# JackAILab/ConsistentID

Hardware: AMD Instinct MI355X
Metric: 512x512 SD1.5 images/sec/node @50 DDIM steps (higher is better)
Workload: dtype f16; 1 GPU; sd15 ConsistentID 512x512, 50 DDIM steps, batch 4/GPU (global 4), CFG batch 8, LoRA rank 128 merged, start_merge_step 30, hipGraph on; global_batch=4, parallelism=dp1 (images sharded, no in-step collective)

## Files before the change

### consistentid_amd/csrc/attn.hip

```cpp
#include "common.h"
#include "../../include/cid.h"
#include <stdlib.h>
#include <type_traits>

#ifndef CID_ATTN_ABL
#define CID_ATTN_ABL 0
#endif
#ifdef CID_ATTN_MAX_AT_HEAD
#define CID_ATTN_HEADMAX true
#else
#define CID_ATTN_HEADMAX false
#endif

namespace {

__device__ __forceinline__ float max17f(float m, const f32x16& v) {
#pragma unroll
    for (int r = 0; r < 16; r += 2) m = __builtin_fmaxf(__builtin_fmaxf(m, v[r]), v[r + 1]);
    return m;
}

template <int D, int QT, int NWV>
struct AttnCfg {
    static constexpr int NT = 64 * NWV;
    static constexpr int BQ = 32 * QT * NWV;
    static constexpr int DKP = (D + 15) / 16 * 16;
    static constexpr int KSTEPS = DKP / 16;
    static constexpr int DVT = (D + 31) / 32;
    static constexpr int NCH = D / 8;
    static constexpr int CR = DVT * 32 - D;
    static constexpr int KBYTES = (DKP / 8) * 1024;
    static constexpr int VDATA = D * 128;
    static constexpr int VBYTES = VDATA + CR * 128;
    static constexpr int BUF = KBYTES + VBYTES;
    static constexpr int PPW = (NCH + NWV - 1) / NWV;
};

template <int D, int QT, int NWV, bool MASK, bool CAUSAL = false>
__global__ void __launch_bounds__(64 * NWV, (QT == 1 && D <= 40 && NWV == 4) ? 3 : ((QT == 1 && D <= 80) ? 2 : 1))
self_attn_kernel(const half_t* __restrict__ q, const half_t* __restrict__ k, const half_t* __restrict__ vt,
                 half_t* __restrict__ out, int N, int heads, int ldq, int ldk, int dvp, int ldo, int n_keys, int xcd_remap) {
#if defined(__HIP_DEVICE_COMPILE__)
    using Cfg = AttnCfg<D, QT, NWV>;
    constexpr int NT = Cfg::NT, KSTEPS = Cfg::KSTEPS, DVT = Cfg::DVT;
    constexpr int NCH = Cfg::NCH, CR = Cfg::CR;
    extern __shared__ __attribute__((aligned(16))) char smem[];
    typedef __attribute__((address_space(3))) void lds_void;

    const int tid = threadIdx.x, lane = tid & 63;
    const int wave = __builtin_amdgcn_readfirstlane(tid >> 6);
    const int idx = lane & 31, hi = lane >> 5;
    int bid = blockIdx.x + gridDim.x * (blockIdx.y + gridDim.y * blockIdx.z);
    {
        const int nwg = gridDim.x * gridDim.y * gridDim.z;
        if (xcd_remap && (nwg & 7) == 0) bid = (bid & 7) * (nwg >> 3) + (bid >> 3);
    }
    const int bx = bid % (int)gridDim.x;
    const int h = (bid / (int)gridDim.x) % (int)gridDim.y, b = bid / (int)(gridDim.x * gridDim.y);
    const int q0 = bx * Cfg::BQ + wave * (32 * QT);

    const half_t* kbase = k + (long)b * N * ldk + h * D;
    const half_t* vbase = vt + ((long)(b * heads + h) * dvp) * N;

#if defined(CID_ATTN_NOBIAS)
    constexpr bool BIAS = false;
#else
    constexpr bool BIAS = Cfg::DKP > D;
#endif
    static_assert(!BIAS || Cfg::DKP - D == 8, "pad is one 16-byte slot");
    static_assert(!(CAUSAL && BIAS), "causal mode: the running max starts behind the mask (no bias slot)");
    if (Cfg::DKP > D) {
        half8 pad = zero_h8();
        if (BIAS) pad[0] = (half_t)1.f;
        for (int r = tid; r < 2 * 64; r += NT)
            *reinterpret_cast<half8*>(smem + (r >> 6) * Cfg::BUF + NCH * 1024 + (r & 63) * 16) = pad;
    }
    const bool bias_lane = BIAS && ((KSTEPS - 1) * 16 + hi * 8 == D);

    half8 qf[QT][KSTEPS];
#pragma unroll
    for (int t = 0; t < QT; ++t) {
        const half_t* qrow = q + ((long)b * N + q0 + t * 32 + idx) * ldq + h * D;
#pragma unroll
        for (int kk = 0; kk < KSTEPS; ++kk) {
            const int c = kk * 16 + hi * 8;
            qf[t][kk] = (c < D) ? ld_global_h8(qrow + c) : zero_h8();
        }
    }

    constexpr bool ONES = (D % 32) != 0;
    constexpr int ONES_REG = ((D % 32) & 3) + 4 * ((D % 32) >> 3);
    constexpr int ONES_HI = ((D % 32) >> 2) & 1;
    if (ONES) {
        half8 one;
#pragma unroll
        for (int i = 0; i < 8; ++i) one[i] = (half_t)1.f;
        for (int e = tid; e < 2 * 8 * CR; e += NT) {
            const int bf = e / (8 * CR), rem = e - bf * (8 * CR);
            *reinterpret_cast<half8*>(smem + bf * Cfg::BUF + Cfg::KBYTES + Cfg::VDATA + rem * 16) = one;
        }
    }

    const __amdgpu_buffer_rsrc_t rs_k = __builtin_amdgcn_make_buffer_rsrc((void*)kbase, 0, (unsigned)(((long)(N - 1) * ldk + D) * 2), 0x00020000);
    const __amdgpu_buffer_rsrc_t rs_v = __builtin_amdgcn_make_buffer_rsrc((void*)vbase, 0, (unsigned)((long)D * N * 2), 0x00020000);
    const unsigned kvo = (unsigned)(lane * ldk * 2);
    unsigned vvo[Cfg::PPW];
#pragma unroll
    for (int j = 0; j < Cfg::PPW; ++j) {
        const int sl = (j * NWV + wave) * 64 + lane;
        const int c = sl / D, r = sl - c * D;
        vvo[j] = (unsigned)(((long)r * N + c * 8) * 2);
    }
    auto dma_k = [&](int key0, int buf) {
#pragma unroll
        for (int j = 0; j < Cfg::PPW; ++j) {
            const int p = j * NWV + wave;
            if (p < NCH)
                __builtin_amdgcn_raw_ptr_buffer_load_lds(rs_k, (lds_void*)(smem + buf * Cfg::BUF + p * 1024), 16, kvo,
                                                         key0 * ldk * 2 + p * 16, 0, 0);
        }
    };
    auto dma_v = [&](int key0, int buf) {
#pragma unroll
        for (int j = 0; j < Cfg::PPW; ++j) {
            const int p = j * NWV + wave;
            if (p < NCH)
                __builtin_amdgcn_raw_ptr_buffer_load_lds(rs_v, (lds_void*)(smem + buf * Cfg::BUF + Cfg::KBYTES + p * 1024), 16,
                                                         vvo[j], key0 * 2, 0, 0);
        }
    };
    auto qk = [&](int buf, f32x16 (&s)[2][QT]) {
        const char* kb = smem + buf * Cfg::BUF;
#pragma unroll
        for (int kt = 0; kt < 2; ++kt)
#pragma unroll
            for (int t = 0; t < QT; ++t) s[kt][t] = zero_f16v();
#pragma unroll
        for (int kk = 0; kk < KSTEPS; ++kk) {
            half8 kf[2];
#pragma unroll
            for (int kt = 0; kt < 2; ++kt)
                kf[kt] = *reinterpret_cast<const half8*>(kb + (kk * 2 + hi) * 1024 + (kt * 32 + idx) * 16);
#pragma unroll
            for (int kt = 0; kt < 2; ++kt)
#pragma unroll
                for (int t = 0; t < QT; ++t) { if (!(CID_ATTN_ABL & 4)) s[kt][t] = mfma32(kf[kt], qf[t][kk], s[kt][t]); else s[kt][t][kk] += (float)kf[kt][0]; }
        }
    };
    const int vlane = (hi * D + idx) * 16;
    const int vlane_c = Cfg::VDATA + (hi * CR + idx + (DVT - 1) * 32 - D) * 16;
    const bool vconst_lane = (DVT - 1) * 32 + idx >= D;

    f32x16 oacc[DVT][QT];
#pragma unroll
    for (int d = 0; d < DVT; ++d)
#pragma unroll
        for (int t = 0; t < QT; ++t) oacc[d][t] = zero_f16v();
    float m_run[QT], l_run[QT];
#pragma unroll
    for (int t = 0; t < QT; ++t) { m_run[t] = -INFINITY; l_run[t] = 0.f; }

    const int ntiles = CAUSAL ? (min(n_keys, bx * Cfg::BQ + Cfg::BQ) + 63) / 64 : N / 64;
    dma_k(0, 0); dma_v(0, 0);
    if (ntiles > 1) dma_k(64, 1);
    asm volatile("s_waitcnt vmcnt(0)" ::: "memory");
    __syncthreads();
    f32x16 s_cur[2][QT], s_nxt[2][QT];
    qk(0, s_cur);
    auto tile_max = [&](f32x16 (&sc)[2][QT], int t) {
        float mx = max17f(sc[0][t][0], sc[0][t]);
        mx = max17f(mx, sc[1][t]);
        return fmaxf(mx, __shfl_xor(mx, 32, 64));
    };
    auto rebias = [&](f32x16 (&sc)[2][QT], int t, float m_new, float delta) {
        if (bias_lane) qf[t][KSTEPS - 1][0] = (half_t)(-m_new);
#pragma unroll
        for (int kt = 0; kt < 2; ++kt)
#pragma unroll
            for (int r = 0; r < 16; ++r) sc[kt][t][r] -= delta;
    };
    float mx_a[QT], mx_b[QT];
    if (MASK && BIAS && n_keys < 64) {
#pragma unroll
        for (int kt = 0; kt < 2; ++kt)
#pragma unroll
            for (int t = 0; t < QT; ++t)
#pragma unroll
                for (int r = 0; r < 16; ++r)
                    if (kt * 32 + crow(r, hi) >= n_keys) s_cur[kt][t][r] = -INFINITY;
    }
#pragma unroll
    for (int t = 0; t < QT; ++t) {
        const float mx = tile_max(s_cur, t);
        if (BIAS) {
            const float m0 = (float)(half_t)fminf(fmaxf(mx, -60000.f), 60000.f);
            rebias(s_cur, t, m0, m0);
            m_run[t] = m0;
            mx_a[t] = mx - m0;
        } else {
            mx_a[t] = mx;
        }
        mx_b[t] = 0.f;
    }
    __syncthreads();

    auto step = [&](int tile, auto has_next_tag, f32x16 (&s_cur)[2][QT], f32x16 (&s_nxt)[2][QT], float (&mx_cur)[QT],
                    float (&mx_nxt)[QT]) {
        constexpr bool HAS_NEXT = decltype(has_next_tag)::value;
        const int cur = tile & 1;
        if (!(CID_ATTN_ABL & 8)) {
            if (tile + 2 < ntiles) dma_k((tile + 2) * 64, cur);
            if (HAS_NEXT) dma_v((tile + 1) * 64, cur ^ 1);
        }
        if (MASK && (tile + 1) * 64 > n_keys) {
#pragma unroll
            for (int kt = 0; kt < 2; ++kt)
#pragma unroll
                for (int t = 0; t < QT; ++t)
#pragma unroll
                    for (int r = 0; r < 16; ++r)
                        if (tile * 64 + kt * 32 + crow(r, hi) >= n_keys) s_cur[kt][t][r] = -INFINITY;
        }
        if (CAUSAL && (tile * 64 + 63 > q0 || (tile + 1) * 64 > n_keys)) {
#pragma unroll
            for (int kt = 0; kt < 2; ++kt)
#pragma unroll
                for (int t = 0; t < QT; ++t)
#pragma unroll
                    for (int r = 0; r < 16; ++r) {
                        const int j = tile * 64 + kt * 32 + crow(r, hi);
                        if (j > q0 + t * 32 + idx || j >= n_keys) s_cur[kt][t][r] = -INFINITY;
                    }
        }
#pragma unroll
        for (int t = 0; t < QT; ++t) {
            const float mx = (CID_ATTN_ABL & 16) ? s_cur[0][t][0] : ((MASK || CAUSAL || CID_ATTN_HEADMAX) ? tile_max(s_cur, t) : mx_cur[t]);
            if (__any(mx > (BIAS ? 8.f : m_run[t] + 8.f))) {
                float m_new, alpha;
                if (BIAS) {
                    m_new = (float)(half_t)fminf(m_run[t] + fmaxf(mx, 0.f), 60000.f);
                    const float delta = m_new - m_run[t];
                    alpha = __builtin_amdgcn_exp2f(-delta);
                    rebias(s_cur, t, m_new, delta);
                } else {
                    m_new = fmaxf(m_run[t], mx);
                    alpha = __builtin_amdgcn_exp2f(m_run[t] - m_new);
                }
                m_run[t] = m_new;
                l_run[t] *= alpha;
#pragma unroll
                for (int d = 0; d < DVT; ++d)
#pragma unroll
                    for (int r = 0; r < 16; ++r) oacc[d][t][r] *= alpha;
            }
        }
        if (HAS_NEXT) qk(cur ^ 1, s_nxt);
        half8 pf[QT][4];
#pragma unroll
        for (int t = 0; t < QT; ++t) {
            const float m = m_run[t];
            float rs = 0.f;
#pragma unroll
            for (int kt = 0; kt < 2; ++kt)
#pragma unroll
                for (int g = 0; g < 2; ++g) {
                    half8 pv;
#pragma unroll
                    for (int i = 0; i < 8; ++i) {
                        const float a_ = BIAS ? s_cur[kt][t][g * 8 + i] : s_cur[kt][t][g * 8 + i] - m;
                        const float p = (CID_ATTN_ABL & 1) ? a_ * 0.001f : __builtin_amdgcn_exp2f(a_);
                        if (!ONES) rs += p;
                        pv[i] = (half_t)p;
                    }
                    pf[t][kt * 2 + g] = pv;
                }
            if (!ONES) l_run[t] += rs;
        }
        const char* vb = smem + cur * Cfg::BUF + Cfg::KBYTES;
#pragma unroll
        for (int ks = 0; ks < 4; ++ks) {
            half8 vf[DVT];
#pragma unroll
            for (int d = 0; d < DVT; ++d) {
                int off = vlane + (ks * 2 * D + d * 32) * 16;
                if (CR > 0 && d == DVT - 1) off = vconst_lane ? vlane_c + ks * 2 * CR * 16 : off;
                vf[d] = *reinterpret_cast<const half8*>(vb + off);
            }
#pragma unroll
            for (int d = 0; d < DVT; ++d)
#pragma unroll
                for (int t = 0; t < QT; ++t) { if (!(CID_ATTN_ABL & 2)) oacc[d][t] = mfma32(vf[d], pf[t][ks], oacc[d][t]); else oacc[d][t][ks] += (float)vf[d][0] * (float)pf[t][ks][0]; }
        }
        if (HAS_NEXT && !MASK && !CAUSAL && !CID_ATTN_HEADMAX) {
#pragma unroll
            for (int t = 0; t < QT; ++t) mx_nxt[t] = tile_max(s_nxt, t);
        }
        asm volatile("s_waitcnt vmcnt(0)" ::: "memory");
        __syncthreads();
    };
    int tile = 0;
    for (; tile + 2 < ntiles; tile += 2) {
        step(tile, std::true_type{}, s_cur, s_nxt, mx_a, mx_b);
        step(tile + 1, std::true_type{}, s_nxt, s_cur, mx_b, mx_a);
    }
    if (ntiles - tile == 2) {
        step(tile, std::true_type{}, s_cur, s_nxt, mx_a, mx_b);
        step(tile + 1, std::false_type{}, s_nxt, s_cur, mx_b, mx_a);
    } else {
        step(tile, std::false_type{}, s_cur, s_nxt, mx_a, mx_b);
    }

#pragma unroll
    for (int t = 0; t < QT; ++t) {
        float l;
        if (ONES) {
            const float mine = oacc[DVT - 1][t][ONES_REG];
            const float other = __shfl_xor(mine, 32, 64);
            l = (hi == ONES_HI) ? mine : other;
        } else {
            l = l_run[t] + __shfl_xor(l_run[t], 32, 64);
        }
        const float inv = 1.f / l;
        half_t* orow = out + ((long)b * N + q0 + t * 32 + idx) * ldo + h * D;
#pragma unroll
        for (int d = 0; d < DVT; ++d)
#pragma unroll
            for (int j = 0; j < 4; ++j) {
                const int dd = d * 32 + 8 * j + 4 * hi;
                if (dd < D) {
                    half4 o;
#pragma unroll
                    for (int i = 0; i < 4; ++i) o[i] = (half_t)(oacc[d][t][j * 4 + i] * inv);
                    *reinterpret_cast<half4*>(orow + dd) = o;
                }
            }
    }
#endif
}

template <int D, int QT, int NWV, bool MASK = false, bool CAUSAL = false>
int launch_attn(const half_t* q, const half_t* k, const half_t* vt, half_t* out, int B, int N, int heads,
                int ldq, int ldk, int dvp, int ldo, int n_keys, hipStream_t s) {
    using Cfg = AttnCfg<D, QT, NWV>;
    constexpr int smem = 2 * Cfg::BUF;
    static bool configured = false;
    auto kern = self_attn_kernel<D, QT, NWV, MASK, CAUSAL>;
    if (!configured) {
        hipError_t herr = hipFuncSetAttribute((const void*)kern, hipFuncAttributeMaxDynamicSharedMemorySize, smem);
        if (herr != hipSuccess) {
            cid_set_error("cid_self_attn_f16: cannot reserve %d bytes of LDS (%s)", smem, hipGetErrorString(herr));
            return -5;
        }
        configured = true;
    }
    dim3 grid(N / Cfg::BQ, heads, B);
    static int remap = -1;
    if (remap < 0) { const char* e = getenv("CID_ATTN_XCD"); remap = e ? atoi(e) : 1; }
    hipLaunchKernelGGL(kern, grid, dim3(Cfg::NT), smem, s, q, k, vt, out, N, heads, ldq, ldk, dvp, ldo, n_keys, remap);
    return 0;
}

}

extern "C" int cid_self_attn_f16(const cid_half* q, const cid_half* k, const cid_half* vt, cid_half* out,
                                 int32_t B, int32_t N, int32_t heads, int32_t d,
                                 int32_t ldq, int32_t ldk, int32_t dvp, int32_t ldo, cid_stream_t stream) {
    return cid_self_attn_keys_f16(q, k, vt, out, B, N, heads, d, ldq, ldk, dvp, ldo, N, stream);
}

extern "C" int cid_self_attn_keys_f16(const cid_half* q, const cid_half* k, const cid_half* vt, cid_half* out,
                                      int32_t B, int32_t N, int32_t heads, int32_t d, int32_t ldq, int32_t ldk,
                                      int32_t dvp, int32_t ldo, int32_t n_keys, cid_stream_t stream) {
    CID_CHECK_ARG(q && k && vt && out, "cid_self_attn_f16: null pointer");
    CID_CHECK_ARG(n_keys > 0 && n_keys <= N, "cid_self_attn_keys_f16: n_keys must be in (0, N] (got %d, N = %d)", n_keys, N);
    CID_CHECK_ARG(B > 0 && heads > 0 && N > 0 && N % 64 == 0, "cid_self_attn_f16: N must be a positive multiple of 64 (got %d)", N);
    CID_CHECK_ARG(ldq % 8 == 0 && ldk % 8 == 0 && ldo % 4 == 0 && dvp >= d, "cid_self_attn_f16: bad pitches");
    const half_t* Q = (const half_t*)q; const half_t* K = (const half_t*)k; const half_t* V = (const half_t*)vt;
    half_t* O = (half_t*)out;
    hipStream_t s = (hipStream_t)stream;
    int rc = -22;
#define CID_ATTN(DD, QT, NWV) rc = launch_attn<DD, QT, NWV>(Q, K, V, O, B, N, heads, ldq, ldk, dvp, ldo, n_keys, s)
#define CID_ATTN_MASKED(DD) \
    rc = (N % 128 == 0) ? launch_attn<DD, 1, 4, true>(Q, K, V, O, B, N, heads, ldq, ldk, dvp, ldo, n_keys, s) \
                        : launch_attn<DD, 1, 2, true>(Q, K, V, O, B, N, heads, ldq, ldk, dvp, ldo, n_keys, s)
    if (n_keys != N) {
        if (d == 80) CID_ATTN_MASKED(80);
        else if (d == 64) CID_ATTN_MASKED(64);
        else if (d == 40) CID_ATTN_MASKED(40);
        else if (d == 160) CID_ATTN_MASKED(160);
        else if (d == 32) CID_ATTN_MASKED(32);
        else { cid_set_error("cid_self_attn_keys_f16: unsupported head dim %d (40, 64, 80, 160, 32)", d); return -22; }
        if (rc) return rc;
        CID_CHECK_LAUNCH("cid_self_attn_keys_f16");
        return 0;
    }
    if (d == 40) {
        if (N % 128 == 0) CID_ATTN(40, 1, 4); else CID_ATTN(40, 1, 2);
    } else if (d == 64 || d == 80) {
        static int force_qt = -1;
        if (force_qt < 0) { const char* e = getenv("CID_ATTN_QT"); force_qt = e ? atoi(e) : 0; }
        const bool qt2 = (N % 256 == 0) && force_qt == 2;
        if (d == 64) {
            if (qt2) CID_ATTN(64, 2, 4); else if (N % 128 == 0) CID_ATTN(64, 1, 4); else CID_ATTN(64, 1, 2);
        } else {
            if (qt2) CID_ATTN(80, 2, 4); else if (N % 128 == 0) CID_ATTN(80, 1, 4); else CID_ATTN(80, 1, 2);
        }
    } else if (d == 160) {
        if (N % 128 == 0) CID_ATTN(160, 1, 4); else CID_ATTN(160, 1, 2);
    } else if (d == 32) {
        if (N % 128 == 0) CID_ATTN(32, 1, 4); else CID_ATTN(32, 1, 2);
    } else {
        cid_set_error("cid_self_attn_f16: unsupported head dim %d (40, 64, 80, 160, 32)", d);
        return -22;
    }
#undef CID_ATTN
#undef CID_ATTN_MASKED
    if (rc) return rc;
    CID_CHECK_LAUNCH("cid_self_attn_f16");
    return 0;
}

extern "C" int cid_self_attn_causal_f16(const cid_half* q, const cid_half* k, const cid_half* vt, cid_half* out,
                                        int32_t B, int32_t N, int32_t heads, int32_t d, int32_t ldq, int32_t ldk,
                                        int32_t dvp, int32_t ldo, int32_t n_keys, cid_stream_t stream) {
    CID_CHECK_ARG(q && k && vt && out, "cid_self_attn_causal_f16: null pointer");
    CID_CHECK_ARG(d == 64, "cid_self_attn_causal_f16: unsupported head dim %d (64)", d);
    CID_CHECK_ARG(B > 0 && heads > 0 && N > 0 && N % 64 == 0, "cid_self_attn_causal_f16: N must be a positive multiple of 64 (got %d)", N);
    CID_CHECK_ARG(n_keys > 0 && n_keys <= N, "cid_self_attn_causal_f16: n_keys must be in (0, N] (got %d, N = %d)", n_keys, N);
    CID_CHECK_ARG(ldq % 8 == 0 && ldk % 8 == 0 && ldo % 4 == 0 && dvp >= d && ldq >= heads * d && ldk >= heads * d &&
                  ldo >= heads * d, "cid_self_attn_causal_f16: bad pitches");
    const int rc = launch_attn<64, 1, 2, false, true>((const half_t*)q, (const half_t*)k, (const half_t*)vt, (half_t*)out, B,
                                                      N, heads, ldq, ldk, dvp, ldo, n_keys, (hipStream_t)stream);
    if (rc) return rc;
    CID_CHECK_LAUNCH("cid_self_attn_causal_f16");
    return 0;
}
```

### consistentid_amd/csrc/norm.hip

```cpp
#include "common.h"
#include "../../include/cid.h"

namespace {

constexpr int LN_MAXCH = 3;

__global__ void __launch_bounds__(256)
layernorm_kernel(const half_t* __restrict__ x, half_t* __restrict__ out,
                 const half_t* __restrict__ gamma, const half_t* __restrict__ beta,
                 int M, int C, long ldx, long ldo, float eps) {
    const int lane = threadIdx.x & 63;
    const int row = blockIdx.x * 4 + (threadIdx.x >> 6);
    if (row >= M) return;
    const int nch = C >> 3;
    const half_t* xr = x + (long)row * ldx;
    float v[LN_MAXCH][8];
    float s = 0.f;
#pragma unroll
    for (int k = 0; k < LN_MAXCH; ++k) {
        const int c = lane + k * 64;
        if (c < nch) {
            const half8 h = ld_global_h8(xr + c * 8);
#pragma unroll
            for (int i = 0; i < 8; ++i) { v[k][i] = (float)h[i]; s += v[k][i]; }
        } else {
#pragma unroll
            for (int i = 0; i < 8; ++i) v[k][i] = 0.f;
        }
    }
    const float mean = wave_sum(s) / (float)C;
    float q = 0.f;
#pragma unroll
    for (int k = 0; k < LN_MAXCH; ++k) {
        const int c = lane + k * 64;
        if (c < nch) {
#pragma unroll
            for (int i = 0; i < 8; ++i) { const float d = v[k][i] - mean; q += d * d; }
        }
    }
    const float rstd = rsqrtf(wave_sum(q) / (float)C + eps);
    half_t* orow = out + (long)row * ldo;
#pragma unroll
    for (int k = 0; k < LN_MAXCH; ++k) {
        const int c = lane + k * 64;
        if (c < nch) {
            const half8 g = ld_global_h8(gamma + c * 8), b = ld_global_h8(beta + c * 8);
            half8 o;
#pragma unroll
            for (int i = 0; i < 8; ++i) o[i] = (half_t)((v[k][i] - mean) * rstd * (float)g[i] + (float)b[i]);
            *reinterpret_cast<half8*>(orow + c * 8) = o;
        }
    }
}

constexpr int LNR_MAXCH = 10;
template <int LPR>
__global__ void __launch_bounds__(256)
layernorm_rows_kernel(const half_t* __restrict__ x, half_t* __restrict__ out,
                      const half_t* __restrict__ gamma, const half_t* __restrict__ beta,
                      int M, int C, long ldx, long ldo, float eps) {
    constexpr int RPW = 64 / LPR;
    const int lane = threadIdx.x & 63;
    const int sub = lane % LPR;
    const int row = (blockIdx.x * 4 + (threadIdx.x >> 6)) * RPW + lane / LPR;
    const int nk = (C >> 3) / LPR;
    const bool live = row < M;
    const half_t* xr = x + (long)(live ? row : 0) * ldx;
    half8 h[LNR_MAXCH], g[LNR_MAXCH], b[LNR_MAXCH];
#pragma unroll
    for (int k = 0; k < LNR_MAXCH; ++k)
        if (k < nk) h[k] = ld_global_h8(xr + (sub + k * LPR) * 8);
#pragma unroll
    for (int k = 0; k < LNR_MAXCH; ++k)
        if (k < nk) { g[k] = ld_global_h8(gamma + (sub + k * LPR) * 8); b[k] = ld_global_h8(beta + (sub + k * LPR) * 8); }
    float s = 0.f;
#pragma unroll
    for (int k = 0; k < LNR_MAXCH; ++k)
        if (k < nk)
#pragma unroll
            for (int i = 0; i < 8; ++i) s += (float)h[k][i];
#pragma unroll
    for (int o = LPR / 2; o > 0; o >>= 1) s += __shfl_xor(s, o, 64);
    const float mean = s / (float)C;
    float q = 0.f;
#pragma unroll
    for (int k = 0; k < LNR_MAXCH; ++k)
        if (k < nk)
#pragma unroll
            for (int i = 0; i < 8; ++i) { const float d = (float)h[k][i] - mean; q += d * d; }
#pragma unroll
    for (int o = LPR / 2; o > 0; o >>= 1) q += __shfl_xor(q, o, 64);
    const float rstd = rsqrtf(q / (float)C + eps);
    if (!live) return;
    half_t* orow = out + (long)row * ldo;
#pragma unroll
    for (int k = 0; k < LNR_MAXCH; ++k)
        if (k < nk) {
            half8 o;
#pragma unroll
            for (int i = 0; i < 8; ++i) o[i] = (half_t)(((float)h[k][i] - mean) * rstd * (float)g[k][i] + (float)b[k][i]);
            *reinterpret_cast<half8*>(orow + (sub + k * LPR) * 8) = o;
        }
}

constexpr int GN_ROWS_PER_BLOCK = 32;
constexpr int GN_MAXC = 2560;
constexpr int GN_MAXBLK = 512;

__global__ void __launch_bounds__(256)
gn_partial_kernel(const half_t* __restrict__ x1, const half_t* __restrict__ x2, int c1, int c2,
                  int HW, int groups, int rows_per_block, float* __restrict__ part ) {
    __shared__ float ssum[GN_MAXC], ssq[GN_MAXC];
    const int C = c1 + c2, nch = C >> 3;
    const int b = blockIdx.y, blk = blockIdx.x, nblk = gridDim.x;
    const int r0 = blk * rows_per_block;
    const int r1 = min(HW, r0 + rows_per_block);
    const int phases = nch <= 256 ? 256 / nch : 1;
    for (int cc0 = 0; cc0 < nch; cc0 += 256) {
        const int t = threadIdx.x;
        const int col = nch <= 256 ? t % nch : cc0 + t;
        const int ph = nch <= 256 ? t / nch : 0;
        if (col < nch && ph < phases) {
            float s[8], q[8];
#pragma unroll
            for (int i = 0; i < 8; ++i) { s[i] = 0.f; q[i] = 0.f; }
            const int ch0 = col * 8;
            const half_t* base; int ld, off;
            if (ch0 < c1) { base = x1; ld = c1; off = ch0; } else { base = x2; ld = c2; off = ch0 - c1; }
            const half_t* p = base + ((long)b * HW) * ld + off;
            int r = r0 + ph;
            for (; r + 7 * phases < r1; r += 8 * phases) {
                half8 h[8];
#pragma unroll
                for (int u = 0; u < 8; ++u) h[u] = ld_global_h8(p + (long)(r + u * phases) * ld);
#pragma unroll
                for (int u = 0; u < 8; ++u)
#pragma unroll
                    for (int i = 0; i < 8; ++i) { const float f = (float)h[u][i]; s[i] += f; q[i] += f * f; }
            }
            for (; r < r1; r += phases) {
                const half8 h = ld_global_h8(p + (long)r * ld);
#pragma unroll
                for (int i = 0; i < 8; ++i) { const float f = (float)h[i]; s[i] += f; q[i] += f * f; }
            }
#pragma unroll
            for (int i = 0; i < 8; ++i) { ssum[ph * C + ch0 + i] = s[i]; ssq[ph * C + ch0 + i] = q[i]; }
        }
    }
    __syncthreads();
    const int cg = C / groups;
    if ((int)threadIdx.x < groups) {
        float s = 0.f, q = 0.f;
        for (int ph = 0; ph < phases; ++ph)
            for (int c = threadIdx.x * cg; c < (threadIdx.x + 1) * cg; ++c) { s += ssum[ph * C + c]; q += ssq[ph * C + c]; }
        float* p = part + (((long)b * nblk + blk) * groups + threadIdx.x) * 2;
        p[0] = s; p[1] = q;
    }
}

template <bool SILU>
__global__ void __launch_bounds__(256)
gn_apply_kernel(const half_t* __restrict__ x1, const half_t* __restrict__ x2, int c1, int c2,
                half_t* __restrict__ out, const float* __restrict__ part, int nblk, int groups, float eps,
                const half_t* __restrict__ gamma, const half_t* __restrict__ beta, int HW, int rows_per_block,
                const float* __restrict__ st1, int nb1, const float* __restrict__ st2, int nb2) {
    __shared__ float sscale[GN_MAXC], sshift[GN_MAXC];
    __shared__ float smean[64], srstd[64];
    __shared__ double dsum[256], dsq[256];
    const int C = c1 + c2, nch = C >> 3;
    const int b = blockIdx.y;
    const int cg = C / groups;
    if (part == nullptr) {
        const int slices = 256 / groups;
        const int g = threadIdx.x % groups, sl = threadIdx.x / groups;
        double s = 0.0, q = 0.0;
        if (sl < slices) {
            const bool first = g * cg < c1;
            const int u = (first ? c1 : c2) >> 5;
            const int upg = cg / u;
            const int u0 = (first ? g * cg : g * cg - c1) / u;
            const int nb = first ? nb1 : nb2;
            const float* st = (first ? st1 : st2) + (long)b * nb * 64;
            for (int k = sl; k < nb * upg; k += slices) {
                const int blk = k / upg, uu = k - blk * upg;
                const float* p = st + ((long)blk * 32 + u0 + uu) * 2;
                s += (double)p[0]; q += (double)p[1];
            }
        }
        dsum[threadIdx.x] = s; dsq[threadIdx.x] = q;
    } else {
        const int slices = 256 / groups;
        const int g = threadIdx.x % groups, sl = threadIdx.x / groups;
        double s = 0.0, q = 0.0;
        if (sl < slices)
            for (int k = sl; k < nblk; k += slices) {
                const float* p = part + (((long)b * nblk + k) * groups + g) * 2;
                s += (double)p[0]; q += (double)p[1];
            }
        dsum[threadIdx.x] = s; dsq[threadIdx.x] = q;
    }
    __syncthreads();
    if ((int)threadIdx.x < groups) {
        const int slices = 256 / groups;
        double s = 0.0, q = 0.0;
        for (int sl = 0; sl < slices; ++sl) { s += dsum[sl * groups + threadIdx.x]; q += dsq[sl * groups + threadIdx.x]; }
        const double n = (double)HW * (double)cg;
        const double mean = s / n;
        double var = q / n - mean * mean;
        if (var < 0.0) var = 0.0;
        smean[threadIdx.x] = (float)mean;
        srstd[threadIdx.x] = (float)(1.0 / sqrt(var + (double)eps));
    }
    __syncthreads();
    for (int c = threadIdx.x; c < C; c += 256) {
        const int g = c / cg;
        const float sc = srstd[g] * (float)gamma[c];
        sscale[c] = sc;
        sshift[c] = (float)beta[c] - smean[g] * sc;
    }
    __syncthreads();
    const int r0 = blockIdx.x * rows_per_block;
    const int r1 = min(HW, r0 + rows_per_block);
    const long total = (long)(r1 - r0) * nch;
    for (long q = threadIdx.x; q < total; q += 256) {
        const int rr = (int)(q / nch);
        const int cc = (int)(q - (long)rr * nch);
        const long row = (long)b * HW + r0 + rr;
        const int ch0 = cc * 8;
        half8 h;
        if (ch0 < c1) h = ld_global_h8(x1 + row * c1 + ch0);
        else          h = ld_global_h8(x2 + row * c2 + (ch0 - c1));
        half8 o;
#pragma unroll
        for (int i = 0; i < 8; ++i) {
            float y = (float)h[i] * sscale[ch0 + i] + sshift[ch0 + i];
            if (SILU) y = silu_f(y);
            o[i] = (half_t)y;
        }
        *reinterpret_cast<half8*>(out + row * C + ch0) = o;
    }
}


constexpr int GNS_MAXPER = 20;
constexpr long GNS_MAXELEM = 256L * GNS_MAXPER * 4;
#ifndef GNS_MAXHW
#define GNS_MAXHW 256
#endif

template <bool SILU>
__global__ void __launch_bounds__(256)
gn_small_kernel(const half_t* __restrict__ x1, const half_t* __restrict__ x2, int c1, int c2, half_t* __restrict__ out,
                const half_t* __restrict__ gamma, const half_t* __restrict__ beta, int B, int HW, int groups, float eps,
                int step_r, int step_c) {
    __shared__ float wsum[4], wsq[4];
    __shared__ float sstat[2];
    const int C = c1 + c2, cg = C / groups, cq = cg >> 2;
    int b, g;
    {
        const int i = blockIdx.x;
        if ((B & 7) == 0) { const int j = i >> 3; b = (i & 7) + 8 * (j / groups); g = j % groups; }
        else { b = i / groups; g = i % groups; }
    }
    const int nchunk = HW * cq;
    const int r_first = (int)threadIdx.x / cq, c_first = (int)threadIdx.x - r_first * cq;
    half4 v[GNS_MAXPER];
    float s = 0.f, q = 0.f;
    int r = r_first, cc = c_first;
#pragma unroll
    for (int k = 0; k < GNS_MAXPER; ++k) {
        const int idx = threadIdx.x + k * 256;
        if (idx < nchunk) {
            const int ch0 = g * cg + 4 * cc;
            const long row = (long)b * HW + r;
            v[k] = ch0 < c1 ? *reinterpret_cast<const half4*>(x1 + row * c1 + ch0)
                            : *reinterpret_cast<const half4*>(x2 + row * c2 + (ch0 - c1));
#pragma unroll
            for (int i = 0; i < 4; ++i) s += (float)v[k][i];
        }
        r += step_r; cc += step_c;
        if (cc >= cq) { cc -= cq; ++r; }
    }
    const double n = (double)HW * (double)cg;
    s = wave_sum(s);
    if ((threadIdx.x & 63) == 0) wsum[threadIdx.x >> 6] = s;
    __syncthreads();
    if (threadIdx.x == 0)
        sstat[0] = (float)(((double)wsum[0] + (double)wsum[1] + (double)wsum[2] + (double)wsum[3]) / n);
    __syncthreads();
    const float mean = sstat[0];
#pragma unroll
    for (int k = 0; k < GNS_MAXPER; ++k) {
        if ((int)threadIdx.x + k * 256 < nchunk) {
#pragma unroll
            for (int i = 0; i < 4; ++i) { const float d = (float)v[k][i] - mean; q = __builtin_fmaf(d, d, q); }
        }
    }
    q = wave_sum(q);
    if ((threadIdx.x & 63) == 0) wsq[threadIdx.x >> 6] = q;
    __syncthreads();
    if (threadIdx.x == 0) {
        const double var = ((double)wsq[0] + (double)wsq[1] + (double)wsq[2] + (double)wsq[3]) / n;
        sstat[1] = (float)(1.0 / sqrt(var + (double)eps));
    }
    __syncthreads();
    const float rstd = sstat[1];
    r = r_first; cc = c_first;
#pragma unroll
    for (int k = 0; k < GNS_MAXPER; ++k) {
        const int idx = threadIdx.x + k * 256;
        if (idx < nchunk) {
            const int ch0 = g * cg + 4 * cc;
            const half4 gm = *reinterpret_cast<const half4*>(gamma + ch0), bt = *reinterpret_cast<const half4*>(beta + ch0);
            half4 o;
#pragma unroll
            for (int i = 0; i < 4; ++i) {
                const float sc = rstd * (float)gm[i];
                float y = (float)v[k][i] * sc + ((float)bt[i] - mean * sc);
                if (SILU) y = silu_f(y);
                o[i] = (half_t)y;
            }
            *reinterpret_cast<half4*>(out + ((long)b * HW + r) * C + ch0) = o;
        }
        r += step_r; cc += step_c;
        if (cc >= cq) { cc -= cq; ++r; }
    }
}

__global__ void __launch_bounds__(256)
softmax_rows_kernel(half_t* __restrict__ x, int rows, int cols, long ld) {
    const int lane = threadIdx.x & 63;
    const long row = (long)blockIdx.x * 4 + (threadIdx.x >> 6);
    if (row >= rows) return;
    half_t* p = x + row * ld;
    const int nch = cols >> 3;
    float mx = -INFINITY;
    for (int c = lane; c < nch; c += 64) {
        const half8 h = ld_global_h8(p + c * 8);
#pragma unroll
        for (int i = 0; i < 8; ++i) mx = fmaxf(mx, (float)h[i]);
    }
#pragma unroll
    for (int o = 32; o > 0; o >>= 1) mx = fmaxf(mx, __shfl_xor(mx, o, 64));
    float s = 0.f;
    for (int c = lane; c < nch; c += 64) {
        const half8 h = ld_global_h8(p + c * 8);
#pragma unroll
        for (int i = 0; i < 8; ++i) s += __builtin_amdgcn_exp2f((float)h[i] - mx);
    }
    const float inv = 1.f / wave_sum(s);
    for (int c = lane; c < nch; c += 64) {
        const half8 h = ld_global_h8(p + c * 8);
        half8 o;
#pragma unroll
        for (int i = 0; i < 8; ++i) o[i] = (half_t)(__builtin_amdgcn_exp2f((float)h[i] - mx) * inv);
        *reinterpret_cast<half8*>(p + c * 8) = o;
    }
}

inline int gn_rows(int HW) { return GN_ROWS_PER_BLOCK * ((HW + GN_ROWS_PER_BLOCK * GN_MAXBLK - 1) / (GN_ROWS_PER_BLOCK * GN_MAXBLK)); }
inline int gn_nblk(int HW) { return (HW + gn_rows(HW) - 1) / gn_rows(HW); }

}

extern "C" int cid_layernorm_ld_f16(const cid_half* x, int64_t ldx, cid_half* out, int64_t ldo, const cid_half* gamma,
                                    const cid_half* beta, int32_t M, int32_t C, float eps, cid_stream_t stream) {
    CID_CHECK_ARG(x && out && gamma && beta, "cid_layernorm_ld_f16: null pointer");
    CID_CHECK_ARG(M > 0 && C > 0 && C % 8 == 0 && C <= 8 * 64 * LN_MAXCH, "cid_layernorm_ld_f16: bad shape M=%d C=%d", M, C);
    CID_CHECK_ARG(ldx >= C && ldo >= C && ldx % 8 == 0 && ldo % 8 == 0, "cid_layernorm_ld_f16: bad pitch ldx=%lld ldo=%lld (C=%d)",
                  (long long)ldx, (long long)ldo, C);
    const int nch = C >> 3;
    const bool big = (long)M * C >= (8L << 20);
    if (!big)
        hipLaunchKernelGGL(layernorm_kernel, dim3((M + 3) / 4), dim3(256), 0, (hipStream_t)stream,
                           (const half_t*)x, (half_t*)out, (const half_t*)gamma, (const half_t*)beta, M, C, (long)ldx, (long)ldo, eps);
    else if (nch % 8 == 0 && nch / 8 <= LNR_MAXCH)
        hipLaunchKernelGGL(layernorm_rows_kernel<8>, dim3((M + 31) / 32), dim3(256), 0, (hipStream_t)stream,
                           (const half_t*)x, (half_t*)out, (const half_t*)gamma, (const half_t*)beta, M, C, (long)ldx, (long)ldo, eps);
    else if (nch % 16 == 0 && nch / 16 <= LNR_MAXCH)
        hipLaunchKernelGGL(layernorm_rows_kernel<16>, dim3((M + 15) / 16), dim3(256), 0, (hipStream_t)stream,
                           (const half_t*)x, (half_t*)out, (const half_t*)gamma, (const half_t*)beta, M, C, (long)ldx, (long)ldo, eps);
    else
        hipLaunchKernelGGL(layernorm_kernel, dim3((M + 3) / 4), dim3(256), 0, (hipStream_t)stream,
                           (const half_t*)x, (half_t*)out, (const half_t*)gamma, (const half_t*)beta, M, C, (long)ldx, (long)ldo, eps);
    CID_CHECK_LAUNCH("cid_layernorm_ld_f16");
    return 0;
}

extern "C" int cid_layernorm_f16(const cid_half* x, cid_half* out, const cid_half* gamma, const cid_half* beta,
                                 int32_t M, int32_t C, float eps, cid_stream_t stream) {
    return cid_layernorm_ld_f16(x, C, out, C, gamma, beta, M, C, eps, stream);
}


extern "C" int cid_softmax_rows_f16(cid_half* x, int32_t rows, int32_t cols, int64_t ld, cid_stream_t stream) {
    CID_CHECK_ARG(x && rows > 0 && cols > 0 && cols % 8 == 0 && ld >= cols && ld % 8 == 0, "cid_softmax_rows_f16: bad shape");
    hipLaunchKernelGGL(softmax_rows_kernel, dim3((rows + 3) / 4), dim3(256), 0, (hipStream_t)stream, (half_t*)x, rows, cols, (long)ld);
    CID_CHECK_LAUNCH("cid_softmax_rows_f16");
    return 0;
}

extern "C" int64_t cid_groupnorm_ws_bytes(int32_t B, int32_t C) {
    (void)C;
    return (int64_t)B * GN_MAXBLK * 64 * 2 * 4;
}

extern "C" int cid_groupnorm_f16(const cid_half* x1, const cid_half* x2, int32_t c1, int32_t c2,
                                 cid_half* out, const cid_half* gamma, const cid_half* beta,
                                 int32_t B, int32_t HW, int32_t groups, float eps, int32_t silu,
                                 void* ws, cid_stream_t stream) {
    CID_CHECK_ARG(x1 && out && gamma && beta && ws, "cid_groupnorm_f16: null pointer");
    const int C = c1 + c2;
    CID_CHECK_ARG(c1 > 0 && c1 % 8 == 0 && c2 >= 0 && c2 % 8 == 0 && (c2 == 0 || x2), "cid_groupnorm_f16: bad channels");
    CID_CHECK_ARG(groups > 0 && groups <= 64 && C % groups == 0 && C <= GN_MAXC, "cid_groupnorm_f16: bad groups/C");
    CID_CHECK_ARG(B > 0 && HW > 0 && HW <= 1024 * 1024, "cid_groupnorm_f16: bad B/HW");
    const int nblk = gn_nblk(HW);
    float* part = (float*)ws;
    hipStream_t s = (hipStream_t)stream;
    const int cg = C / groups;
    if (cg % 4 == 0 && HW <= GNS_MAXHW && (long)HW * cg <= GNS_MAXELEM) {
        const int cq = cg / 4;
        if (silu)
            hipLaunchKernelGGL(gn_small_kernel<true>, dim3(groups * B), dim3(256), 0, s, (const half_t*)x1, (const half_t*)x2, c1, c2,
                               (half_t*)out, (const half_t*)gamma, (const half_t*)beta, B, HW, groups, eps, 256 / cq, 256 % cq);
        else
            hipLaunchKernelGGL(gn_small_kernel<false>, dim3(groups * B), dim3(256), 0, s, (const half_t*)x1, (const half_t*)x2, c1, c2,
                               (half_t*)out, (const half_t*)gamma, (const half_t*)beta, B, HW, groups, eps, 256 / cq, 256 % cq);
        CID_CHECK_LAUNCH("cid_groupnorm_f16");
        return 0;
    }
    hipLaunchKernelGGL(gn_partial_kernel, dim3(nblk, B), dim3(256), 0, s,
                       (const half_t*)x1, (const half_t*)x2, c1, c2, HW, groups, gn_rows(HW), part);
    int rpb = (16384 / (C * 2)) > 0 ? 16384 / (C * 2) : 1;
    if ((HW + rpb - 1) / rpb > 1024) rpb = (HW + 1023) / 1024;
    if (rpb > HW) rpb = HW;
    const int ablk = (HW + rpb - 1) / rpb;
    if (silu)
        hipLaunchKernelGGL(gn_apply_kernel<true>, dim3(ablk, B), dim3(256), 0, s, (const half_t*)x1, (const half_t*)x2,
                           c1, c2, (half_t*)out, part, nblk, groups, eps, (const half_t*)gamma, (const half_t*)beta, HW, rpb,
                           (const float*)nullptr, 0, (const float*)nullptr, 0);
    else
        hipLaunchKernelGGL(gn_apply_kernel<false>, dim3(ablk, B), dim3(256), 0, s, (const half_t*)x1, (const half_t*)x2,
                           c1, c2, (half_t*)out, part, nblk, groups, eps, (const half_t*)gamma, (const half_t*)beta, HW, rpb,
                           (const float*)nullptr, 0, (const float*)nullptr, 0);
    CID_CHECK_LAUNCH("cid_groupnorm_f16");
    return 0;
}

extern "C" int cid_groupnorm_stats_ok(int32_t c1, int32_t c2, int32_t groups) {
    const int C = c1 + c2;
    if (groups <= 0 || groups > 64 || C % groups || c1 <= 0 || c1 % 32 || c2 < 0 || c2 % 32) return 0;
    const int cg = C / groups;
    if (c1 % cg) return 0;
    if (cg % (c1 / 32)) return 0;
    if (c2 && cg % (c2 / 32)) return 0;
    return 1;
}

extern "C" int cid_groupnorm_stats_f16(const cid_half* x1, const cid_half* x2, int32_t c1, int32_t c2,
                                       cid_half* out, const cid_half* gamma, const cid_half* beta,
                                       int32_t B, int32_t HW, int32_t groups, float eps, int32_t silu,
                                       const float* stats1, int32_t rows1, const float* stats2, int32_t rows2,
                                       cid_stream_t stream) {
    CID_CHECK_ARG(x1 && out && gamma && beta && stats1, "cid_groupnorm_stats_f16: null pointer");
    const int C = c1 + c2;
    CID_CHECK_ARG(c1 > 0 && c1 % 8 == 0 && c2 >= 0 && c2 % 8 == 0 && (c2 == 0 || (x2 && stats2)), "cid_groupnorm_stats_f16: bad channels");
    CID_CHECK_ARG(C <= GN_MAXC && cid_groupnorm_stats_ok(c1, c2, groups),
                  "cid_groupnorm_stats_f16: groups of %d channels are not whole statistics units of one source (c1=%d c2=%d)",
                  groups ? C / groups : 0, c1, c2);
    CID_CHECK_ARG(B > 0 && HW > 0 && rows1 > 0 && HW % rows1 == 0 && (c2 == 0 || (rows2 > 0 && HW % rows2 == 0)),
                  "cid_groupnorm_stats_f16: a statistics block must lie inside one sample (HW=%d rows %d / %d)", HW, rows1, rows2);
    hipStream_t s = (hipStream_t)stream;
    int rpb = (16384 / (C * 2)) > 0 ? 16384 / (C * 2) : 1;
    if ((HW + rpb - 1) / rpb > 1024) rpb = (HW + 1023) / 1024;
    if (rpb > HW) rpb = HW;
    const int ablk = (HW + rpb - 1) / rpb;
    const int nb1 = HW / rows1, nb2 = c2 ? HW / rows2 : 0;
    if (silu)
        hipLaunchKernelGGL(gn_apply_kernel<true>, dim3(ablk, B), dim3(256), 0, s, (const half_t*)x1, (const half_t*)x2,
                           c1, c2, (half_t*)out, (const float*)nullptr, 0, groups, eps, (const half_t*)gamma, (const half_t*)beta,
                           HW, rpb, stats1, nb1, stats2, nb2);
    else
        hipLaunchKernelGGL(gn_apply_kernel<false>, dim3(ablk, B), dim3(256), 0, s, (const half_t*)x1, (const half_t*)x2,
                           c1, c2, (half_t*)out, (const float*)nullptr, 0, groups, eps, (const half_t*)gamma, (const half_t*)beta,
                           HW, rpb, stats1, nb1, stats2, nb2);
    CID_CHECK_LAUNCH("cid_groupnorm_stats_f16");
    return 0;
}
```

Before: 7.801 images/s.

## Pick attention query tile by CU fill; widen small-groupnorm to 1024 threads

Attention now uses the 128-row query tile only when the grid of 128-row tiles covers at least the device's CU count, and otherwise falls back to 64-row tiles to get more blocks on small problems. The small-groupnorm kernel is rewritten to run 1024 threads per block, use 8-wide half loads when pointers are aligned, and preload gamma and beta. It also drops the single-thread double reduction and its extra barriers, and precomputes the inverse element count on the host. This adds more template instantiations and switches rstd to a float rsqrt, which slightly changes precision.

```diff
diff --git a/consistentid_amd/csrc/attn.hip b/consistentid_amd/csrc/attn.hip
--- a/consistentid_amd/csrc/attn.hip
+++ b/consistentid_amd/csrc/attn.hip
@@ -360,6 +360,23 @@
     return 0;
 }
 
+int attn_bq128(int B, int N, int heads) {
+    if (N % 128 != 0) return 0;
+    static int force = -1, cus = 0;
+    if (force < 0) { const char* e = getenv("CID_ATTN_BQ"); force = e ? atoi(e) : 0; }
+    if (force == 128 || force == 64) return force == 128;
+    if (cus <= 0) {
+        int dev = 0, n = 0;
+        if (hipGetDevice(&dev) != hipSuccess || hipDeviceGetAttribute(&n, hipDeviceAttributeMultiprocessorCount, dev) != hipSuccess ||
+            n <= 0) {
+            cid_set_error("cid_self_attn_f16: cannot read the device's CU count");
+            return -1;
+        }
+        cus = n;
+    }
+    return (long)(N / 128) * heads * B >= cus;
+}
+
 }
 
 extern "C" int cid_self_attn_f16(const cid_half* q, const cid_half* k, const cid_half* vt, cid_half* out,
@@ -379,9 +396,12 @@
     half_t* O = (half_t*)out;
     hipStream_t s = (hipStream_t)stream;
     int rc = -22;
+    const int bq = (d == 40 || d == 64 || d == 80 || d == 160 || d == 32) ? attn_bq128(B, N, heads) : 0;
+    if (bq < 0) return -5;
+    const bool bq128 = bq == 1;
 #define CID_ATTN(DD, QT, NWV) rc = launch_attn<DD, QT, NWV>(Q, K, V, O, B, N, heads, ldq, ldk, dvp, ldo, n_keys, s)
 #define CID_ATTN_MASKED(DD) \
-    rc = (N % 128 == 0) ? launch_attn<DD, 1, 4, true>(Q, K, V, O, B, N, heads, ldq, ldk, dvp, ldo, n_keys, s) \
+    rc = bq128 ? launch_attn<DD, 1, 4, true>(Q, K, V, O, B, N, heads, ldq, ldk, dvp, ldo, n_keys, s) \
                         : launch_attn<DD, 1, 2, true>(Q, K, V, O, B, N, heads, ldq, ldk, dvp, ldo, n_keys, s)
     if (n_keys != N) {
         if (d == 80) CID_ATTN_MASKED(80);
@@ -395,20 +415,20 @@
         return 0;
     }
     if (d == 40) {
-        if (N % 128 == 0) CID_ATTN(40, 1, 4); else CID_ATTN(40, 1, 2);
+        if (bq128) CID_ATTN(40, 1, 4); else CID_ATTN(40, 1, 2);
     } else if (d == 64 || d == 80) {
         static int force_qt = -1;
         if (force_qt < 0) { const char* e = getenv("CID_ATTN_QT"); force_qt = e ? atoi(e) : 0; }
         const bool qt2 = (N % 256 == 0) && force_qt == 2;
         if (d == 64) {
-            if (qt2) CID_ATTN(64, 2, 4); else if (N % 128 == 0) CID_ATTN(64, 1, 4); else CID_ATTN(64, 1, 2);
+            if (qt2) CID_ATTN(64, 2, 4); else if (bq128) CID_ATTN(64, 1, 4); else CID_ATTN(64, 1, 2);
         } else {
-            if (qt2) CID_ATTN(80, 2, 4); else if (N % 128 == 0) CID_ATTN(80, 1, 4); else CID_ATTN(80, 1, 2);
+            if (qt2) CID_ATTN(80, 2, 4); else if (bq128) CID_ATTN(80, 1, 4); else CID_ATTN(80, 1, 2);
         }
     } else if (d == 160) {
-        if (N % 128 == 0) CID_ATTN(160, 1, 4); else CID_ATTN(160, 1, 2);
+        if (bq128) CID_ATTN(160, 1, 4); else CID_ATTN(160, 1, 2);
     } else if (d == 32) {
-        if (N % 128 == 0) CID_ATTN(32, 1, 4); else CID_ATTN(32, 1, 2);
+        if (bq128) CID_ATTN(32, 1, 4); else CID_ATTN(32, 1, 2);
     } else {
         cid_set_error("cid_self_attn_f16: unsupported head dim %d (40, 64, 80, 160, 32)", d);
         return -22;
diff --git a/consistentid_amd/csrc/norm.hip b/consistentid_amd/csrc/norm.hip
--- a/consistentid_amd/csrc/norm.hip
+++ b/consistentid_amd/csrc/norm.hip
@@ -242,20 +242,29 @@
 }
 
 
-constexpr int GNS_MAXPER = 20;
-constexpr long GNS_MAXELEM = 256L * GNS_MAXPER * 4;
+constexpr long GNS_MAXELEM = 20480;
 #ifndef GNS_MAXHW
 #define GNS_MAXHW 256
 #endif
-
-template <bool SILU>
-__global__ void __launch_bounds__(256)
+#ifndef GNS_THREADS
+#define GNS_THREADS 1024
+#endif
+constexpr int gns_per(int nt, int e) { return (int)((GNS_MAXELEM + nt * e - 1) / (nt * e)); }
+
+template <int E> struct GnsVec;
+template <> struct GnsVec<4> { using type = half4; };
+template <> struct GnsVec<8> { using type = half8; };
+
+template <bool SILU, int NT, int E>
+__global__ void __launch_bounds__(NT)
 gn_small_kernel(const half_t* __restrict__ x1, const half_t* __restrict__ x2, int c1, int c2, half_t* __restrict__ out,
                 const half_t* __restrict__ gamma, const half_t* __restrict__ beta, int B, int HW, int groups, float eps,
-                int step_r, int step_c) {
-    __shared__ float wsum[4], wsq[4];
-    __shared__ float sstat[2];
-    const int C = c1 + c2, cg = C / groups, cq = cg >> 2;
+                int step_r, int step_c,
+                double inv_n) {
+    using vec_t = typename GnsVec<E>::type;
+    constexpr int PER = gns_per(NT, E), NW = NT / 64;
+    __shared__ float wsum[NW], wsq[NW];
+    const int C = c1 + c2, cg = C / groups, cq = cg / E;
     int b, g;
     {
         const int i = blockIdx.x;
@@ -264,63 +273,71 @@
     }
     const int nchunk = HW * cq;
     const int r_first = (int)threadIdx.x / cq, c_first = (int)threadIdx.x - r_first * cq;
-    half4 v[GNS_MAXPER];
-    float s = 0.f, q = 0.f;
+    vec_t v[PER], gm[PER], bt[PER];
     int r = r_first, cc = c_first;
 #pragma unroll
-    for (int k = 0; k < GNS_MAXPER; ++k) {
-        const int idx = threadIdx.x + k * 256;
-        if (idx < nchunk) {
-            const int ch0 = g * cg + 4 * cc;
+    for (int k = 0; k < PER; ++k) {
+        if ((int)threadIdx.x + k * NT < nchunk) {
+            const int ch0 = g * cg + E * cc;
             const long row = (long)b * HW + r;
-            v[k] = ch0 < c1 ? *reinterpret_cast<const half4*>(x1 + row * c1 + ch0)
-                            : *reinterpret_cast<const half4*>(x2 + row * c2 + (ch0 - c1));
-#pragma unroll
-            for (int i = 0; i < 4; ++i) s += (float)v[k][i];
+            v[k] = ch0 < c1 ? *reinterpret_cast<const vec_t*>(x1 + row * c1 + ch0)
+                            : *reinterpret_cast<const vec_t*>(x2 + row * c2 + (ch0 - c1));
         }
         r += step_r; cc += step_c;
         if (cc >= cq) { cc -= cq; ++r; }
     }
-    const double n = (double)HW * (double)cg;
+    cc = c_first;
+#pragma unroll
+    for (int k = 0; k < PER; ++k) {
+        if ((int)threadIdx.x + k * NT < nchunk) {
+            gm[k] = *reinterpret_cast<const vec_t*>(gamma + g * cg + E * cc);
+            bt[k] = *reinterpret_cast<const vec_t*>(beta + g * cg + E * cc);
+        }
+        cc += step_c;
+        if (cc >= cq) cc -= cq;
+    }
+    float s = 0.f, q = 0.f;
+#pragma unroll
+    for (int k = 0; k < PER; ++k) {
+        if ((int)threadIdx.x + k * NT < nchunk) {
+#pragma unroll
+            for (int i = 0; i < E; ++i) s += (float)v[k][i];
+        }
+    }
     s = wave_sum(s);
     if ((threadIdx.x & 63) == 0) wsum[threadIdx.x >> 6] = s;
     __syncthreads();
-    if (threadIdx.x == 0)
-        sstat[0] = (float)(((double)wsum[0] + (double)wsum[1] + (double)wsum[2] + (double)wsum[3]) / n);
-    __syncthreads();
-    const float mean = sstat[0];
-#pragma unroll
-    for (int k = 0; k < GNS_MAXPER; ++k) {
-        if ((int)threadIdx.x + k * 256 < nchunk) {
-#pragma unroll
-            for (int i = 0; i < 4; ++i) { const float d = (float)v[k][i] - mean; q = __builtin_fmaf(d, d, q); }
+    double ts = 0.0;
+#pragma unroll
+    for (int w = 0; w < NW; ++w) ts += (double)wsum[w];
+    const float mean = (float)(ts * inv_n);
+#pragma unroll
+    for (int k = 0; k < PER; ++k) {
+        if ((int)threadIdx.x + k * NT < nchunk) {
+#pragma unroll
+            for (int i = 0; i < E; ++i) { const float d = (float)v[k][i] - mean; q = __builtin_fmaf(d, d, q); }
         }
     }
     q = wave_sum(q);
     if ((threadIdx.x & 63) == 0) wsq[threadIdx.x >> 6] = q;
     __syncthreads();
-    if (threadIdx.x == 0) {
-        const double var = ((double)wsq[0] + (double)wsq[1] + (double)wsq[2] + (double)wsq[3]) / n;
-        sstat[1] = (float)(1.0 / sqrt(var + (double)eps));
-    }
-    __syncthreads();
-    const float rstd = sstat[1];
+    double tq = 0.0;
+#pragma unroll
+    for (int w = 0; w < NW; ++w) tq += (double)wsq[w];
+    const float rstd = rsqrtf((float)(tq * inv_n) + eps);
     r = r_first; cc = c_first;
 #pragma unroll
-    for (int k = 0; k < GNS_MAXPER; ++k) {
-        const int idx = threadIdx.x + k * 256;
-        if (idx < nchunk) {
-            const int ch0 = g * cg + 4 * cc;
-            const half4 gm = *reinterpret_cast<const half4*>(gamma + ch0), bt = *reinterpret_cast<const half4*>(beta + ch0);
-            half4 o;
-#pragma unroll
-            for (int i = 0; i < 4; ++i) {
-                const float sc = rstd * (float)gm[i];
-                float y = (float)v[k][i] * sc + ((float)bt[i] - mean * sc);
+    for (int k = 0; k < PER; ++k) {
+        if ((int)threadIdx.x + k * NT < nchunk) {
+            vec_t o;
+#pragma unroll
+            for (int i = 0; i < E; ++i) {
+                const float sc = rstd * (float)gm[k][i];
+                float y = (float)v[k][i] * sc + ((float)bt[k][i] - mean * sc);
                 if (SILU) y = silu_f(y);
                 o[i] = (half_t)y;
             }
-            *reinterpret_cast<half4*>(out + ((long)b * HW + r) * C + ch0) = o;
+            *reinterpret_cast<vec_t*>(out + ((long)b * HW + r) * C + g * cg + E * cc) = o;
         }
         r += step_r; cc += step_c;
         if (cc >= cq) { cc -= cq; ++r; }
@@ -419,13 +436,17 @@
     hipStream_t s = (hipStream_t)stream;
     const int cg = C / groups;
     if (cg % 4 == 0 && HW <= GNS_MAXHW && (long)HW * cg <= GNS_MAXELEM) {
-        const int cq = cg / 4;
-        if (silu)
-            hipLaunchKernelGGL(gn_small_kernel<true>, dim3(groups * B), dim3(256), 0, s, (const half_t*)x1, (const half_t*)x2, c1, c2,
-                               (half_t*)out, (const half_t*)gamma, (const half_t*)beta, B, HW, groups, eps, 256 / cq, 256 % cq);
-        else
-            hipLaunchKernelGGL(gn_small_kernel<false>, dim3(groups * B), dim3(256), 0, s, (const half_t*)x1, (const half_t*)x2, c1, c2,
-                               (half_t*)out, (const half_t*)gamma, (const half_t*)beta, B, HW, groups, eps, 256 / cq, 256 % cq);
+        const uintptr_t ptrs = (uintptr_t)x1 | (uintptr_t)x2 | (uintptr_t)out | (uintptr_t)gamma | (uintptr_t)beta;
+        const bool wide = cg % 8 == 0 && ptrs % 16 == 0;
+        const int cq = cg / (wide ? 8 : 4);
+        const double inv_n = 1.0 / ((double)HW * (double)cg);
+        constexpr int NT = GNS_THREADS;
+#define CID_GNS(SILU, E) hipLaunchKernelGGL((gn_small_kernel<SILU, NT, E>), dim3(groups * B), dim3(NT), 0, s, (const half_t*)x1, \
+                                            (const half_t*)x2, c1, c2, (half_t*)out, (const half_t*)gamma, (const half_t*)beta, B, HW, \
+                                            groups, eps, NT / cq, NT % cq, inv_n)
+        if (wide) { if (silu) CID_GNS(true, 8); else CID_GNS(false, 8); }
+        else      { if (silu) CID_GNS(true, 4); else CID_GNS(false, 4); }
+#undef CID_GNS
         CID_CHECK_LAUNCH("cid_groupnorm_f16");
         return 0;
     }
```

Result: faster. 7.902 images/s, median of 6 (+1.3%).
